# AlgoLab/rs-vgaligner

Measured on AMD Instinct MI355X. Metric: aligned reads/sec (10 kbp ONT vs HLA graph), higher is better.
Workload: dtype int32+f64

## Files before the change

rs-vgaligner_amd/csrc/vga_common.hpp:

```cpp
#pragma once

#include <hip/hip_runtime.h>
#include <sys/mman.h>

#include <chrono>
#include <cstdarg>
#include <cstdint>
#include <cstdio>
#include <cstdlib>
#include <cstring>
#include <atomic>
#include <memory>
#include <mutex>
#include <new>
#include <string>
#include <thread>
#include <vector>

#include "../../include/vga_hip.h"
#include "vga_probe_hash.hpp"

#define VGA_ABI_VERSION 6

template <typename T>
// ... 5 lines not shown
}

struct cov_state;
struct ps_state;
struct pu_state;
struct poa_ws;

struct vga_dev_index {
    uint32_t k = 0;
    uint64_t seq_length = 0;
    uint64_t n_nodes = 0, n_edges = 0;
    uint32_t *d_table = nullptr;
    uint64_t table_entries = 0;
    uint2 *d_pos = nullptr;
    uint64_t n_pos_words = 0;
    uint32_t *d_table_all = nullptr;
    uint2 *d_pos_all = nullptr;
    vga_hash_slot *d_hash = nullptr;
    uint32_t hash_mask = 0;
    bool all_view = false;
    uint64_t probe_table_bytes = 0, probe_pos_bytes = 0;
    char *d_seq_fwd = nullptr;
    uint32_t *d_node_start = nullptr, *d_edge_idx = nullptr, *d_edges_to = nullptr, *d_edges = nullptr;
    std::vector<char> seq_fwd;
    std::vector<uint32_t> node_start;
    std::vector<uint32_t> edge_idx;
    std::vector<uint32_t> edges_to;
    std::vector<uint32_t> edges;
    bool loaded = false;
    vga_owned<cov_state> cov{nullptr, nullptr};
    vga_owned<ps_state> ps{nullptr, nullptr};
    vga_owned<pu_state> pu{nullptr, nullptr};
};

struct vga_timer_entry {
    const char *name;
    hipEvent_t e0, e1;
    uint64_t bytes;
    hipStream_t stream;
};

struct vga_deferred { void *dev, *pinned, *reg; size_t reg_bytes; };

struct vga_ctx {
    int device = 0;
    hipStream_t stream = nullptr;
// ... 207 lines not shown
```

rs-vgaligner_amd/csrc/vga_ctx.hip:

```cpp
#include "vga_common.hpp"

#include <mutex>

#include <algorithm>

#include <malloc.h>

int vga_set_error(vga_ctx *ctx, int code, const char *fmt, ...)
{
    char buf[1024];
    va_list ap;
    va_start(ap, fmt);
    vsnprintf(buf, sizeof buf, fmt, ap);
    va_end(ap);
    if (ctx) { std::lock_guard<std::mutex> lk(ctx->err_mu); ctx->err = buf; }
    return code;
}

unsigned vga_host_threads(uint64_t n)
{
    unsigned nt = std::thread::hardware_concurrency();
    if (nt == 0) nt = 4;
    if (nt > 32) nt = 32;
    const char *e = getenv("VGA_HOST_THREADS");
// ... 93 lines not shown
    }
    vga_ctx *ctx = new vga_ctx();
    ctx->device = device;
    if (hipSetDevice(device) != hipSuccess) { delete ctx; return VGA_ERR_NO_DEVICE; }
    if (hipStreamCreateWithFlags(&ctx->stream, hipStreamNonBlocking) != hipSuccess) { delete ctx; return VGA_ERR_HIP; }
    hipDeviceProp_t prop;
    if (hipGetDeviceProperties(&prop, device) == hipSuccess) ctx->n_cu = prop.multiProcessorCount;
    *out = ctx;
    return VGA_OK;
}

void vga_index_release(vga_dev_index &ix)
{
    if (ix.d_table) (void)hipFree(ix.d_table);
    if (ix.d_pos) (void)hipFree(ix.d_pos);
    if (ix.d_table_all) (void)hipFree(ix.d_table_all);
    if (ix.d_pos_all) (void)hipFree(ix.d_pos_all);
    if (ix.d_hash) (void)hipFree(ix.d_hash);
    if (ix.d_seq_fwd) (void)hipFree(ix.d_seq_fwd);
    if (ix.d_node_start) (void)hipFree(ix.d_node_start);
    if (ix.d_edge_idx) (void)hipFree(ix.d_edge_idx);
    if (ix.d_edges_to) (void)hipFree(ix.d_edges_to);
    if (ix.d_edges) (void)hipFree(ix.d_edges);
    ix.cov.reset();
    ix.ps.reset();
    ix.pu.reset();
    ix = vga_dev_index();
}

extern "C" void vga_ctx_destroy(vga_ctx *ctx)
{
    if (!ctx) return;
    (void)hipSetDevice(ctx->device);
    vga_ctx_scope scope(ctx);
    if (ctx->stream) (void)hipStreamSynchronize(ctx->stream);
    for (vga_batch *b : ctx->batches) {
        if (b->d_reads) (void)hipFree(b->d_reads);
        if (b->d_read_off) (void)hipFree(b->d_read_off);
        if (b->d_read_off2) (void)hipFree(b->d_read_off2);
        b->d_reads = nullptr;
        b->d_read_off = nullptr;
        b->d_read_off2 = nullptr;
        b->ctx = nullptr;
    }
    ctx->map_ws.reset();
    ctx->poa_ws.reset();
// ... 129 lines not shown
    ix.seq_fwd.assign(d->seq_fwd, d->seq_fwd + d->seq_length);
    ix.node_start.resize(d->n_nodes + 1);
    ix.edge_idx.resize(d->n_nodes + 1);
    ix.edges_to.resize(d->n_nodes + 1);
    for (uint64_t i = 0; i <= d->n_nodes; i++) {
        ix.node_start[i] = (uint32_t)d->node_seq_idx[i];
        ix.edge_idx[i] = (uint32_t)d->node_edge_idx[i];
        ix.edges_to[i] = (uint32_t)d->node_edges_to[i];
    }
    ix.edges.resize(d->n_edges);
    for (uint64_t i = 0; i < d->n_edges; i++) ix.edges[i] = (uint32_t)d->edges[i];
    const size_t nn1 = (size_t)d->n_nodes + 1;
    VGA_HIP_CHECK(ctx, hipMalloc((void **)&ix.d_seq_fwd, d->seq_length + 16));
    VGA_HIP_CHECK(ctx, hipMalloc((void **)&ix.d_node_start, nn1 * sizeof(uint32_t)));
    VGA_HIP_CHECK(ctx, hipMalloc((void **)&ix.d_edge_idx, nn1 * sizeof(uint32_t)));
    VGA_HIP_CHECK(ctx, hipMalloc((void **)&ix.d_edges_to, nn1 * sizeof(uint32_t)));
    VGA_HIP_CHECK(ctx, hipMalloc((void **)&ix.d_edges, (d->n_edges + 1) * sizeof(uint32_t)));
    VGA_HIP_CHECK(ctx, hipMemcpyAsync(ix.d_seq_fwd, ix.seq_fwd.data(), d->seq_length, hipMemcpyHostToDevice, ctx->stream));
    VGA_HIP_CHECK(ctx, hipMemcpyAsync(ix.d_node_start, ix.node_start.data(), nn1 * sizeof(uint32_t), hipMemcpyHostToDevice, ctx->stream));
    VGA_HIP_CHECK(ctx, hipMemcpyAsync(ix.d_edge_idx, ix.edge_idx.data(), nn1 * sizeof(uint32_t), hipMemcpyHostToDevice, ctx->stream));
    VGA_HIP_CHECK(ctx, hipMemcpyAsync(ix.d_edges_to, ix.edges_to.data(), nn1 * sizeof(uint32_t), hipMemcpyHostToDevice, ctx->stream));
    if (d->n_edges)
        VGA_HIP_CHECK(ctx, hipMemcpyAsync(ix.d_edges, ix.edges.data(), d->n_edges * sizeof(uint32_t), hipMemcpyHostToDevice, ctx->stream));
    VGA_HIP_CHECK(ctx, hipStreamSynchronize(ctx->stream));
    return VGA_OK;
}

__global__ __launch_bounds__(256) void k_probe_hash_insert(const uint64_t *__restrict__ keys, const uint32_t *__restrict__ hdr_all,
                                                           const uint32_t *__restrict__ hdr_ff, uint64_t n, vga_hash_slot *slots,
                                                           uint32_t mask, uint32_t *n_failed)
{
    const uint64_t g = (uint64_t)blockIdx.x * blockDim.x + threadIdx.x;
    if (g >= n) return;
    const uint64_t key = keys[g];
    const uint32_t ha = hdr_all[g];
    uint32_t s = vga_hash_first_slot(key, mask);
    for (uint64_t tries = 0; tries <= mask; tries++, s = vga_hash_next_slot(s, mask)) {
        if (atomicCAS(&slots[s].hdr_all, VGA_HASH_EMPTY, ha) != VGA_HASH_EMPTY) continue;
        slots[s].key = key;
        slots[s].hdr_ff = hdr_ff[g];
        return;
    }
    atomicAdd(n_failed, 1u);
}

static int vga_index_upload_impl(vga_ctx *ctx, const vga_index_desc *d)
// ... 271 lines not shown
```

rs-vgaligner_amd/csrc/vga_subgraph.hip:

```cpp
#include "vga_subgraph.hpp"

#include <algorithm>
#include <string>
#include <vector>

namespace {

#define SG_RING_SPAN 32u

struct sg_index {
    const uint32_t *node_start, *edge_idx, *edges_to, *edges;
    const char *seq;
    uint32_t n_nodes;
};

__device__ __forceinline__ uint32_t sg_ld(const uint32_t *p) { return __hip_atomic_load(p, __ATOMIC_RELAXED, __HIP_MEMORY_SCOPE_AGENT); }

__device__ inline uint32_t sg_rank(const sg_index &ix, uint32_t pos)
{
    uint32_t lo = 0, hi = ix.n_nodes + 1;
    while (lo < hi) {
        const uint32_t mid = (lo + hi) >> 1;
        if (ix.node_start[mid] <= pos) lo = mid + 1; else hi = mid;
    }
    return lo;
}
__device__ inline uint32_t sg_select(const sg_index &ix, uint32_t element_no)
{
    if (element_no == 0 || element_no > ix.n_nodes + 1) return 0;
    return ix.node_start[element_no - 1];
}
__device__ inline uint32_t sg_len(const sg_index &ix, uint32_t h)
{
    const uint32_t id = h >> 1;
    return ix.node_start[id] - ix.node_start[id - 1];
}
template <typename F>
__device__ inline void sg_for_nb(const sg_index &ix, uint32_t h, bool incoming, F f)
{
    const uint32_t pos = (h >> 1) - 1;
    const bool inc = (h & 1u) ? !incoming : incoming;
    const uint32_t s0 = ix.edge_idx[pos], nin = ix.edges_to[pos];
    const uint32_t s = inc ? s0 : s0 + nin, e = inc ? s0 + nin : ix.edge_idx[pos + 1];
    const uint32_t fl = h & 1u;
    for (uint32_t i = s; i < e; i++) f(ix.edges[i] ^ fl);
}

__device__ inline bool sg_member(const uint32_t *bm, uint32_t nh, uint32_t x) { return x < nh && ((sg_ld(bm + (x >> 5)) >> (x & 31u)) & 1u); }

__device__ inline uint32_t wave_sum(uint32_t v)
{
#pragma unroll
    for (int o = 32; o > 0; o >>= 1) v += (uint32_t)__shfl_xor((int)v, o);
    return v;
}
__device__ inline uint32_t wave_max(uint32_t v)
{
#pragma unroll
    for (int o = 32; o > 0; o >>= 1) { const uint32_t t = (uint32_t)__shfl_xor((int)v, o); v = t > v ? t : v; }
    return v;
}
__device__ inline uint32_t wave_min(uint32_t v)
{
#pragma unroll
    for (int o = 32; o > 0; o >>= 1) { const uint32_t t = (uint32_t)__shfl_xor((int)v, o); v = t < v ? t : v; }
    return v;
}
__device__ inline unsigned long long wave_sum64(unsigned long long v)
{
#pragma unroll
    for (int o = 32; o > 0; o >>= 1)
        v += ((unsigned long long)(uint32_t)__shfl_xor((int)(v >> 32), o) << 32) | (uint32_t)__shfl_xor((int)(uint32_t)v, o);
    return v;
}
__device__ inline uint32_t wave_excl(uint32_t v, int lane, uint32_t *total)
{
    uint32_t s = v;
#pragma unroll
    for (int o = 1; o < 64; o <<= 1) {
        const uint32_t t = (uint32_t)__shfl_up((int)s, o);
        if (lane >= o) s += t;
    }
    *total = (uint32_t)__shfl((int)s, 63);
    return s - v;
}

struct sg_node_counts {
    uint32_t len, deg;
    bool has_out;
};
__device__ inline sg_node_counts sg_count_node(const sg_index &ix, const uint32_t *bm, uint32_t nh, uint32_t h)
{
    sg_node_counts c;
    c.len = sg_len(ix, h);
    c.deg = 0;
    c.has_out = false;
    sg_for_nb(ix, h, true, [&](uint32_t x) { if (x < h && sg_member(bm, nh, x)) c.deg++; });
    sg_for_nb(ix, h, false, [&](uint32_t y) { if (y > h && sg_member(bm, nh, y)) c.has_out = true; });
    return c;
}

__device__ void sg_extend(const sg_index &ix, uint32_t from, uint32_t diff, bool incoming, uint32_t *best, uint32_t *stamp,
                          uint32_t *q0, uint32_t *q1, uint32_t *touched, uint32_t &level, uint32_t *s_cnt, uint32_t *s_touched, int lane)
{
    auto relax = [&](uint32_t x, uint32_t rem, uint32_t lvl, uint32_t *q, uint32_t *qn) {
        const uint32_t old = atomicMax(best + x, rem);
        if (old < rem) {
            if (old == 0) touched[atomicAdd(s_touched, 1u)] = x;
            if (atomicExch(stamp + x, lvl) != lvl) q[atomicAdd(qn, 1u)] = x;
        }
    };
    if (lane == 0) { s_cnt[0] = 0; s_cnt[1] = 0; }
    __syncthreads();
    level++;
    if (lane == 0) sg_for_nb(ix, from, incoming, [&](uint32_t x) { relax(x, diff, level, q0, s_cnt); });
    int cq = 0;
    for (;;) {
        __syncthreads();
        const uint32_t cnt = s_cnt[cq];
        if (cnt == 0) break;
        __syncthreads();
        if (lane == 0) s_cnt[cq ^ 1] = 0;
        __syncthreads();
        level++;
        uint32_t *q = cq ? q1 : q0, *qo = cq ? q0 : q1;
        for (uint32_t i = (uint32_t)lane; i < cnt; i += 64) {
            const uint32_t h = sg_ld(q + i);
            const uint32_t left = sg_ld(best + h);
            const uint32_t len = sg_len(ix, h);
            if (len < left) {
                const uint32_t rem = left - len;
                sg_for_nb(ix, h, incoming, [&](uint32_t x) { relax(x, rem, level, qo, s_cnt + (cq ^ 1)); });
            }
        }
        cq ^= 1;
    }
}

__global__ __launch_bounds__(64) void k_sg_mark(const sg_desc *__restrict__ descs, uint32_t n, sg_index ix, uint32_t k, uint32_t words,
                                                uint32_t nh, uint32_t *bitmaps, uint32_t *scratch, sg_sum *sums)
{
    __shared__ uint32_t s_cnt[2], s_touched;
    const int lane = threadIdx.x;
    uint32_t *best = scratch + (uint64_t)blockIdx.x * 5ull * nh, *stamp = best + nh, *q0 = stamp + nh, *q1 = q0 + nh, *touched = q1 + nh;
    for (uint32_t i = (uint32_t)lane; i < nh; i += 64) { best[i] = 0; stamp[i] = 0; }
    uint32_t level = 0;
    __syncthreads();
    for (uint32_t p = blockIdx.x; p < n; p += gridDim.x) {
        const sg_desc d = descs[p];
        uint32_t *bm = bitmaps + (uint64_t)p * words;
        const uint32_t min_id = sg_rank(ix, d.pmin), max_id = sg_rank(ix, d.pmax);
        const uint32_t first_handle = min_id * 2, last_handle = max_id * 2;
        for (uint32_t w = (uint32_t)lane; w < words; w += 64) {
            const uint32_t lo = w * 32u, hi = lo + 31u;
            uint32_t m = 0;
            if (hi >= first_handle && lo <= last_handle) {
                m = 0x55555555u;
                if (first_handle > lo) m &= ~0u << (first_handle - lo);
                if (last_handle < hi) m &= ~0u >> (hi - last_handle);
            }
            bm[w] = m;
        }
        if (lane == 0) s_touched = 0;
        __syncthreads();
        uint32_t prefix_diff = d.q_first;
// ... 8 lines not shown
                atomicOr(bm + (h >> 5), 1u << (h & 31u));
                best[h] = 0;
                wlo = min(wlo, h >> 5);
                whi = max(whi, h >> 5);
            }
            __syncthreads();
            if (lane == 0) s_touched = 0;
            __syncthreads();
        };
        if (prefix_diff > 0) {
            sg_extend(ix, first_handle, prefix_diff, true, best, stamp, q0, q1, touched, level, s_cnt, &s_touched, lane);
            harvest();
        }
        uint32_t suffix_diff = d.qlen - (d.q_last + k);
        const uint32_t end_suffix_on_node = sg_select(ix, (last_handle >> 1) + 1) - 1 - (d.te_last - 1);
        if (end_suffix_on_node > suffix_diff) suffix_diff = 0; else suffix_diff -= end_suffix_on_node;
        if (suffix_diff > 0) {
            sg_extend(ix, last_handle, suffix_diff, false, best, stamp, q0, q1, touched, level, s_cnt, &s_touched, lane);
            harvest();
        }
        wlo = wave_min(wlo);
        whi = wave_max(whi);
        __syncthreads();
        uint32_t c_nodes = 0, c_preds = 0, c_sinks = 0, bad = 0;
        unsigned long long c_rows = 0;
        for (uint32_t w = wlo + (uint32_t)lane; w <= whi; w += 64) {
            uint32_t bits = sg_ld(bm + w);
            while (bits) {
                const uint32_t h = w * 32u + (uint32_t)__builtin_ctz(bits);
                bits &= bits - 1;
                const sg_node_counts c = sg_count_node(ix, bm, nh, h);
                c_nodes++;
                c_rows += c.len;
                c_preds += c.deg ? c.deg : 1u;
                c_sinks += c.has_out ? 0u : 1u;
                if (c.deg > 255 || c.len == 0 || c.len >= (1u << 24)) bad = 1;
            }
        }
        c_nodes = wave_sum(c_nodes);
        c_preds = wave_sum(c_preds);
        c_sinks = wave_sum(c_sinks);
        bad = wave_max(bad);
        const unsigned long long rows = wave_sum64(c_rows);
        if (rows >= (1ull << 31)) bad = 1;
        if (lane == 0) {
            sg_sum s = {};
            s.n_nodes = c_nodes; s.N = (uint32_t)rows; s.n_preds = c_preds; s.n_sinks = c_sinks; s.wlo = wlo; s.whi = whi; s.flags = bad;
            sums[p] = s;
        }
        __syncthreads();
    }
}

__device__ inline char sg_complement(char c)
{
    switch (c) {
    case 'a': return 't'; case 'c': return 'g'; case 't': return 'a'; case 'g': return 'c'; case 'u': return 'a';
    case 'A': return 'T'; case 'C': return 'G'; case 'T': return 'A'; case 'G': return 'C'; case 'U': return 'A';
    default: return 'N';
    }
}

__global__ __launch_bounds__(64) void k_sg_emit(uint32_t n, sg_index ix, uint32_t words, uint32_t nh, const uint32_t *bitmaps, uint32_t *scratch,
                                                sg_sum *sums, const sg_off *__restrict__ offs, uint32_t *handles, uint32_t *first_row, uint4 *ntab,
                                                uint32_t *preds, uint32_t *sinks, char *seq, int first_edge)
{
    const int lane = threadIdx.x;
    uint32_t *wb_rank = scratch + (uint64_t)blockIdx.x * 5ull * nh, *wb_row = wb_rank + words, *wb_pred = wb_row + words, *wb_sink = wb_pred + words;
    uint32_t *rf = scratch + (uint64_t)blockIdx.x * 5ull * nh + nh;
    for (uint32_t p = blockIdx.x; p < n; p += gridDim.x) {
        const sg_sum sm = sums[p];
        if (sm.flags & 1u) continue;
        const sg_off of = offs[p];
        const uint32_t *bm = bitmaps + (uint64_t)p * words;
        const uint32_t wlo = sm.wlo, whi = sm.whi, n_sub = sm.n_nodes;
        uint32_t *hd = handles + of.node0, *fr = first_row + of.node0, *pl = preds + of.pred0, *sl = sinks + of.sink0;
        uint4 *nt = ntab + of.node0 + p;
        char *sq = seq + of.seq0;
        {
            uint32_t run_rank = 0, run_row = 0, run_pred = 0, run_sink = 0;
            for (uint32_t w0 = wlo; w0 <= whi; w0 += 64) {
                const uint32_t w = w0 + (uint32_t)lane;
                uint32_t bits = w <= whi ? bm[w] : 0u;
                uint32_t cn = 0, cr = 0, cp = 0, cs = 0;
                while (bits) {
                    const uint32_t h = w * 32u + (uint32_t)__builtin_ctz(bits);
                    bits &= bits - 1;
                    const sg_node_counts c = sg_count_node(ix, bm, nh, h);
                    cn++; cr += c.len; cp += c.deg ? c.deg : 1u; cs += c.has_out ? 0u : 1u;
                }
                uint32_t tn, tr, tp, ts;
                const uint32_t en = wave_excl(cn, lane, &tn), er = wave_excl(cr, lane, &tr), ep = wave_excl(cp, lane, &tp), es = wave_excl(cs, lane, &ts);
                if (w <= whi) {
                    wb_rank[w - wlo] = run_rank + en; wb_row[w - wlo] = run_row + er; wb_pred[w - wlo] = run_pred + ep; wb_sink[w - wlo] = run_sink + es;
                }
                run_rank += tn; run_row += tr; run_pred += tp; run_sink += ts;
            }
        }
        __syncthreads();
        auto rank_of = [&](uint32_t x) -> uint32_t {
            const uint32_t w = x >> 5;
            return sg_ld(wb_rank + (w - wlo)) + (uint32_t)__builtin_popcount(bm[w] & ((1u << (x & 31u)) - 1u));
        };
        for (uint32_t w = wlo + (uint32_t)lane; w <= whi; w += 64) {
            uint32_t bits = bm[w];
            uint32_t i = sg_ld(wb_rank + (w - wlo)), row = sg_ld(wb_row + (w - wlo));
            while (bits) {
                const uint32_t h = w * 32u + (uint32_t)__builtin_ctz(bits);
                bits &= bits - 1;
                const uint32_t id = h >> 1, s = ix.node_start[id - 1], e = ix.node_start[id];
                hd[i] = h;
                fr[i] = row + 1;
                if (!(h & 1u)) for (uint32_t t = s; t < e; t++) sq[row + (t - s)] = ix.seq[t];
                else for (uint32_t t = e; t-- > s;) sq[row + (e - 1 - t)] = sg_complement(ix.seq[t]);
                row += e - s;
                i++;
            }
        }
        __syncthreads();
        uint32_t life = 1;
        for (uint32_t w = wlo + (uint32_t)lane; w <= whi; w += 64) {
            uint32_t bits = bm[w];
            uint32_t i = sg_ld(wb_rank + (w - wlo)), pcur = sg_ld(wb_pred + (w - wlo)), scur = sg_ld(wb_sink + (w - wlo));
            while (bits) {
                const uint32_t h = w * 32u + (uint32_t)__builtin_ctz(bits);
                bits &= bits - 1;
                const uint32_t len = sg_len(ix, h), frow = sg_ld(fr + i);
                uint32_t deg = 0, last_v = 0, last_k = 0, first_pred = 0;
                bool have_last = false;
                for (;;) {
                    uint32_t best_v = 0xFFFFFFFFu, best_k = 0xFFFFFFFFu, kk = 0;
                    sg_for_nb(ix, h, true, [&](uint32_t x) {
                        const uint32_t kx = kk++;
                        if (!(x < h && sg_member(bm, nh, x))) return;
                        if (have_last && (x < last_v || (x == last_v && kx <= last_k))) return;
                        if (x < best_v || (x == best_v && kx < best_k)) { best_v = x; best_k = kx; }
                    });
                    if (best_k == 0xFFFFFFFFu) break;
                    const uint32_t r = rank_of(best_v);
                    const uint32_t lrow = sg_ld(fr + r) + sg_len(ix, best_v) - 1;
                    pl[pcur + deg] = lrow;
                    if (deg == 0) first_pred = lrow;
                    deg++;
                    last_v = best_v; last_k = best_k; have_last = true;
                }
                if (deg == 0) pl[pcur] = 0;
                uint32_t reach = 0;
                bool has_out = false;
                sg_for_nb(ix, h, false, [&](uint32_t y) {
                    if (y > h && sg_member(bm, nh, y)) { has_out = true; const uint32_t sp = rank_of(y) - i; reach = sp > reach ? sp : reach; }
                });
                if (!has_out) sl[scur++] = frow + len - 1;
                if (reach <= SG_RING_SPAN) life = reach > life ? reach : life;
                nt[1 + i] = make_uint4(frow, len | ((deg ? deg : 1u) << 24), (has_out ? 0u : 0x80000000u) | (reach > SG_RING_SPAN ? 0x40000000u : 0u),
                                       deg <= 1 ? first_pred : pcur);
                pcur += deg ? deg : 1u;
                i++;
            }
        }
        life = wave_max(life);
        __syncthreads();
        uint32_t longest = 0, first_src = 0xFFFFFFFFu;
        for (uint32_t g0 = 0; g0 < n_sub; g0 += 64) {
            const uint32_t top = n_sub - 1 - g0;
            const bool valid = (uint32_t)lane <= top;
            const uint32_t i = valid ? top - (uint32_t)lane : 0u;
            uint32_t val = 0, len = 1;
            unsigned long long mask = 0;
            if (valid) {
                const uint32_t h = sg_ld(hd + i);
                len = sg_len(ix, h);
                bool taken = false;
                sg_for_nb(ix, h, false, [&](uint32_t y) {
                    if (!(y > h && sg_member(bm, nh, y))) return;
                    if (first_edge && taken) return;
                    taken = true;
                    const uint32_t j = rank_of(y);
                    if (j > top) { const uint32_t c = 1u + sg_ld(rf + j); val = c > val ? c : val; }
                    else mask |= 1ull << (top - j);
                });
            }
            for (int s = 0; s < 64; s++) {
                const uint32_t rfs = (uint32_t)__shfl((int)(val + len - 1), s);
                if ((mask >> s) & 1ull) { const uint32_t c = 1u + rfs; val = c > val ? c : val; }
            }
            if (valid) {
                rf[i] = val + len - 1;
                uint32_t *z = (uint32_t *)(nt + 1 + i);
                const uint32_t y = sg_ld(z + 1), wv = sg_ld(z + 3), zf = sg_ld(z + 2);
                z[2] = zf | val;
                if ((y >> 24) == 1u && wv == 0u) {
                    const uint32_t c = 1u + val + len - 1;
                    if (first_edge) { if (i < first_src) { first_src = i; longest = c; } }
                    else longest = c > longest ? c : longest;
                }
            }
            __syncthreads();
        }
        if (first_edge) {
            const uint32_t fs = wave_min(first_src);
            longest = wave_max(first_src == fs && fs != 0xFFFFFFFFu ? longest : 0u);
        } else
            longest = wave_max(longest);
        if (lane == 0) {
            nt[0] = make_uint4(0u, 1u, longest, 0u);
            sums[p].longest = longest;
            sums[p].life = life;
            if (longest >= (1u << 30)) sums[p].flags = 1u;
        }
        __syncthreads();
    }
}

struct sg_part_bufs {
    vga_dbuf<uint32_t> d_handles, d_first_row, d_preds, d_sinks;
    vga_dbuf<uint4> d_ntab;
    vga_dbuf<char> d_seq;
    vga_hbuf<uint32_t> h_handles, h_first_row;
};
struct sg_ws {
    vga_dbuf<sg_desc> d_desc;
    vga_dbuf<sg_sum> d_sum;
    vga_dbuf<sg_off> d_off;
    vga_dbuf<uint32_t> d_bitmaps, d_scratch;
    vga_hbuf<sg_desc> h_desc;
    vga_hbuf<sg_sum> h_sum;
    vga_hbuf<sg_off> h_off;
    sg_part_bufs part[2];
    std::vector<uint64_t> q_src;
    std::string dump;
    std::vector<uint64_t> read_no;
    hipStream_t side = nullptr;
    uint64_t waves = 0;
    uint32_t nh = 0, words = 0;
    ~sg_ws()
    {
        if (side) (void)hipStreamDestroy(side);
    }
};

int sg_dump_part(vga_ctx *ctx, sg_ws &W, const sg_part_bufs &B, uint64_t p0, uint64_t p1, uint64_t tn, uint64_t tp, uint64_t ts, uint64_t tq, hipStream_t st)
{
    const uint64_t n = p1 - p0;
    std::vector<uint4> ntab(tn + n);
    std::vector<uint32_t> preds(tp + 1), sinks(ts + 1);
    std::vector<char> seq(tq + 4);
    VGA_HIP_CHECK_OOM(ctx, hipMemcpyAsync(ntab.data(), B.d_ntab.p, (tn + n) * sizeof(uint4), hipMemcpyDeviceToHost, st));
    if (tp) VGA_HIP_CHECK_OOM(ctx, hipMemcpyAsync(preds.data(), B.d_preds.p, tp * sizeof(uint32_t), hipMemcpyDeviceToHost, st));
    if (ts) VGA_HIP_CHECK_OOM(ctx, hipMemcpyAsync(sinks.data(), B.d_sinks.p, ts * sizeof(uint32_t), hipMemcpyDeviceToHost, st));
    if (tq) VGA_HIP_CHECK_OOM(ctx, hipMemcpyAsync(seq.data(), B.d_seq.p, tq, hipMemcpyDeviceToHost, st));
    VGA_HIP_CHECK_OOM(ctx, hipStreamSynchronize(st));
    FILE *f = fopen(W.dump.c_str(), "a");
    if (!f) return vga_set_error(ctx, VGA_ERR_ARG, "VGA_SG_DUMP: cannot append to %s", W.dump.c_str());
    auto list = [&](const char *tag, const uint32_t *v, uint64_t cnt) {
        fputs(tag, f);
        for (uint64_t i = 0; i < cnt; i++) fprintf(f, " %u", v[i]);
        fputc('\n', f);
// ... 8 lines not shown
        if (s.flags & 1u) continue;
        const uint4 *nt = ntab.data() + o.node0 + (p - p0);
        for (uint32_t i = 0; i <= s.n_nodes; i++)
            fprintf(f, "T %u %u %u %u %u %u %u %u\n", i, nt[i].x, nt[i].y & 0xFFFFFFu, nt[i].y >> 24, nt[i].z >> 31, (nt[i].z >> 30) & 1u, nt[i].z & 0x3FFFFFFFu, nt[i].w);
        list("H", B.h_handles.p + o.node0, s.n_nodes);
        list("F", B.h_first_row.p + o.node0, s.n_nodes);
        list("L", preds.data() + o.pred0, s.n_preds);
        list("K", sinks.data() + o.sink0, s.n_sinks);
        fputs("Q ", f);
        for (uint32_t i = 0; i < s.N; i++) fprintf(f, "%02x", (unsigned)(unsigned char)seq[o.seq0 + i]);
        fputs("\nE\n", f);
    }
    fclose(f);
    return VGA_OK;
}

int sg_run_part(vga_ctx *ctx, sg_ws &W, sg_store &store, int k, uint64_t p0, uint64_t p1, hipStream_t st)
{
    sg_part &P = store.part[k];
    P.p0 = p0; P.p1 = p1;
    if (p1 <= p0) { P.ready = true; return VGA_OK; }
    const uint64_t n = p1 - p0;
    const vga_dev_index &dix = ctx->index;
    sg_index ix = {dix.d_node_start, dix.d_edge_idx, dix.d_edges_to, dix.d_edges, dix.d_seq_fwd, (uint32_t)dix.n_nodes};
    const uint32_t nh = W.nh, words = W.words;
    uint32_t waves = (uint32_t)std::min<uint64_t>(W.waves, n);
    if (k == 1) {
        uint32_t side_waves = 2u * (uint32_t)ctx->n_cu;
        if (const char *e = getenv("VGA_SG_SIDE_WAVES")) side_waves = (uint32_t)std::max(1, atoi(e));
        waves = std::min(waves, side_waves);
    }
    sg_part_bufs &B = W.part[k];
    int t_mark = vga_timer_begin(ctx, "subgraph_mark", 0, st);
    hipLaunchKernelGGL(k_sg_mark, dim3(waves), dim3(64), 0, st, W.d_desc.p + p0, (uint32_t)n, ix, dix.k, words, nh, W.d_bitmaps.p + p0 * words,
                       W.d_scratch.p, W.d_sum.p + p0);
    vga_timer_end(ctx, t_mark);
    VGA_HIP_CHECK_OOM(ctx, hipGetLastError());
    VGA_HIP_CHECK_OOM(ctx, hipMemcpyAsync(W.h_sum.p + p0, W.d_sum.p + p0, n * sizeof(sg_sum), hipMemcpyDeviceToHost, st));
    VGA_HIP_CHECK_OOM(ctx, hipStreamSynchronize(st));
    uint64_t tn = 0, tp = 0, ts = 0, tq = 0;
    for (uint64_t p = p0; p < p1; p++) {
        const sg_sum &s = W.h_sum.p[p];
        sg_off &o = W.h_off.p[p];
        o.node0 = tn; o.pred0 = tp; o.sink0 = ts; o.seq0 = tq; o.q_src = W.q_src[p];
        if (s.flags & 1u) continue;
        tn += s.n_nodes; tp += s.n_preds; ts += s.n_sinks; tq += ((uint64_t)s.N + 3) & ~3ull;
    }
    VGA_HIP_CHECK_OOM(ctx, B.d_handles.reserve(tn + 1)); VGA_HIP_CHECK_OOM(ctx, B.d_first_row.reserve(tn + 1)); VGA_HIP_CHECK_OOM(ctx, B.d_ntab.reserve(tn + n));
    VGA_HIP_CHECK_OOM(ctx, B.d_preds.reserve(tp + 1)); VGA_HIP_CHECK_OOM(ctx, B.d_sinks.reserve(ts + 1)); VGA_HIP_CHECK_OOM(ctx, B.d_seq.reserve(tq + 4));
    VGA_HIP_CHECK_OOM(ctx, B.h_handles.reserve(tn + 1)); VGA_HIP_CHECK_OOM(ctx, B.h_first_row.reserve(tn + 1));
    VGA_HIP_CHECK_OOM(ctx, hipMemcpyAsync(W.d_off.p + p0, W.h_off.p + p0, n * sizeof(sg_off), hipMemcpyHostToDevice, st));
    int t_emit = vga_timer_begin(ctx, "subgraph_emit", 0, st);
    hipLaunchKernelGGL(k_sg_emit, dim3(waves), dim3(64), 0, st, (uint32_t)n, ix, words, nh, W.d_bitmaps.p + p0 * words, W.d_scratch.p, W.d_sum.p + p0,
                       W.d_off.p + p0, B.d_handles.p, B.d_first_row.p, B.d_ntab.p, B.d_preds.p, B.d_sinks.p, B.d_seq.p,
                       store.remain_rule == VGA_REMAIN_FIRST_OUT_EDGE ? 1 : 0);
    vga_timer_end(ctx, t_emit);
    VGA_HIP_CHECK_OOM(ctx, hipGetLastError());
    VGA_HIP_CHECK_OOM(ctx, hipMemcpyAsync(W.h_sum.p + p0, W.d_sum.p + p0, n * sizeof(sg_sum), hipMemcpyDeviceToHost, st));
    if (tn) {
        VGA_HIP_CHECK_OOM(ctx, hipMemcpyAsync(B.h_handles.p, B.d_handles.p, tn * sizeof(uint32_t), hipMemcpyDeviceToHost, st));
        VGA_HIP_CHECK_OOM(ctx, hipMemcpyAsync(B.h_first_row.p, B.d_first_row.p, tn * sizeof(uint32_t), hipMemcpyDeviceToHost, st));
    }
    VGA_HIP_CHECK_OOM(ctx, hipStreamSynchronize(st));
    if (!W.dump.empty()) {
        const int rc = sg_dump_part(ctx, W, B, p0, p1, tn, tp, ts, tq, st);
        if (rc != VGA_OK) return rc;
    }
    P.d_ntab = B.d_ntab.p; P.d_preds = B.d_preds.p; P.d_sinks = B.d_sinks.p; P.d_seq = B.d_seq.p;
    P.d_handles = B.d_handles.p;
    P.h_handles = B.h_handles.p; P.h_first_row = B.h_first_row.p;
    P.ready = true;
    return VGA_OK;
}

}

int sg_prepare(vga_ctx *ctx, const sg_desc *descs, const uint64_t *q_src, const uint64_t *read_no, uint64_t n, uint64_t split, const char *d_reads,
               int remain_rule, sg_store &store)
// ... 3 lines not shown
    if (n == 0) return VGA_OK;
    if (n >= (1ull << 31)) return vga_set_error(ctx, VGA_ERR_UNSUPPORTED, "too many chains in one call");
    (void)hipSetDevice(ctx->device);
    hipStream_t st = ctx->stream;
    if (!ctx->sg_ws && !(ctx->sg_ws = vga_make_owned<void, sg_ws>())) throw std::bad_alloc();
    sg_ws &W = *(sg_ws *)ctx->sg_ws.get();
    if (!W.side) {
        int lo = 0, hi = 0;
        (void)hipDeviceGetStreamPriorityRange(&lo, &hi);
        (void)hi;
        VGA_HIP_CHECK_OOM(ctx, hipStreamCreateWithPriority(&W.side, hipStreamNonBlocking, lo));
    }
    const vga_dev_index &dix = ctx->index;
    W.nh = 2u * ((uint32_t)dix.n_nodes + 2u);
    W.words = (W.nh + 31u) / 32u;
    uint64_t waves = std::min<uint64_t>(n, 16ull * (uint64_t)ctx->n_cu);
    const uint64_t slab = 5ull * W.nh * sizeof(uint32_t);
    W.waves = std::max<uint64_t>(1, std::min<uint64_t>(waves, (4ull << 30) / slab));
    if (split > n) split = n;
    VGA_HIP_CHECK_OOM(ctx, W.d_desc.reserve(n)); VGA_HIP_CHECK_OOM(ctx, W.d_sum.reserve(n)); VGA_HIP_CHECK_OOM(ctx, W.d_off.reserve(n));
    VGA_HIP_CHECK_OOM(ctx, W.h_desc.reserve(n)); VGA_HIP_CHECK_OOM(ctx, W.h_sum.reserve(n)); VGA_HIP_CHECK_OOM(ctx, W.h_off.reserve(n));
    VGA_HIP_CHECK_OOM(ctx, W.d_bitmaps.reserve(n * W.words));
    VGA_HIP_CHECK_OOM(ctx, W.d_scratch.reserve(W.waves * 5ull * W.nh));
    memcpy(W.h_desc.p, descs, n * sizeof(sg_desc));
    W.q_src.assign(q_src, q_src + n);
    const char *dump = getenv("VGA_SG_DUMP");
    W.dump = dump ? dump : "";
    if (!W.dump.empty()) {
        W.read_no.assign(read_no, read_no + n);
        FILE *f = fopen(W.dump.c_str(), "w");
        if (!f) return vga_set_error(ctx, VGA_ERR_ARG, "VGA_SG_DUMP: cannot write %s", W.dump.c_str());
        fclose(f);
    }
    VGA_HIP_CHECK_OOM(ctx, hipMemcpyAsync(W.d_desc.p, W.h_desc.p, n * sizeof(sg_desc), hipMemcpyHostToDevice, st));
    store.n = n;
    store.split = split;
    store.sum = W.h_sum.p; store.off = W.h_off.p; store.d_off = W.d_off.p;
    store.d_reads = d_reads;
    store.part[1].p0 = split; store.part[1].p1 = n;
    return sg_run_part(ctx, W, store, 0, 0, split, st);
}

int sg_prepare_rest(vga_ctx *ctx, sg_store &store)
{
    if (store.part[1].ready) return VGA_OK;
    (void)hipSetDevice(ctx->device);
// ... 4 lines not shown
```

Measured before the change: 10610.

## Pack per-node records, cache bitmap window in LDS, reuse mark prefix sums in emit

Builds a packed 16-byte per-node record (length and edge ranges) and a presorted incoming-edge list at index load, so each node's data comes from one vector load and predecessor emission can scan sorted edges instead of repeatedly searching for the minimum. The mark kernel stages the subgraph bitmap window in shared memory and writes per-word prefix counts to a side buffer, which the emit kernel reuses rather than recounting. Emit also splits sequence copying into a separate coalesced word-wise pass and caches single-successor ranks for the reach pass. The cost is extra device memory for the side buffer and tables, plus a fallback path for windows that exceed the shared-memory size.

Result: no change. 10620 (median of 2 runs) (+0.1%).

```diff
diff --git a/rs-vgaligner_amd/csrc/vga_common.hpp b/rs-vgaligner_amd/csrc/vga_common.hpp
--- a/rs-vgaligner_amd/csrc/vga_common.hpp
+++ b/rs-vgaligner_amd/csrc/vga_common.hpp
@@ -51,6 +51,8 @@
     uint64_t probe_table_bytes = 0, probe_pos_bytes = 0;
     char *d_seq_fwd = nullptr;
     uint32_t *d_node_start = nullptr, *d_edge_idx = nullptr, *d_edges_to = nullptr, *d_edges = nullptr;
+    uint4 *d_sg_rec = nullptr;
+    uint32_t *d_edges_in_sorted = nullptr;
     std::vector<char> seq_fwd;
     std::vector<uint32_t> node_start;
     std::vector<uint32_t> edge_idx;
diff --git a/rs-vgaligner_amd/csrc/vga_ctx.hip b/rs-vgaligner_amd/csrc/vga_ctx.hip
--- a/rs-vgaligner_amd/csrc/vga_ctx.hip
+++ b/rs-vgaligner_amd/csrc/vga_ctx.hip
@@ -1,4 +1,5 @@
 #include "vga_common.hpp"
+#include "vga_sg_tables.hpp"
 
 #include <mutex>
 
@@ -139,6 +140,8 @@
     if (ix.d_edge_idx) (void)hipFree(ix.d_edge_idx);
     if (ix.d_edges_to) (void)hipFree(ix.d_edges_to);
     if (ix.d_edges) (void)hipFree(ix.d_edges);
+    if (ix.d_sg_rec) (void)hipFree(ix.d_sg_rec);
+    if (ix.d_edges_in_sorted) (void)hipFree(ix.d_edges_in_sorted);
     ix.cov.reset();
     ix.ps.reset();
     ix.pu.reset();
@@ -314,6 +317,15 @@
     VGA_HIP_CHECK(ctx, hipMemcpyAsync(ix.d_edges_to, ix.edges_to.data(), nn1 * sizeof(uint32_t), hipMemcpyHostToDevice, ctx->stream));
     if (d->n_edges)
         VGA_HIP_CHECK(ctx, hipMemcpyAsync(ix.d_edges, ix.edges.data(), d->n_edges * sizeof(uint32_t), hipMemcpyHostToDevice, ctx->stream));
+    if (ix.edge_idx[d->n_nodes] > d->n_edges) return vga_set_error(ctx, VGA_ERR_ARG, "node_edge_idx runs past the %llu edges", (unsigned long long)d->n_edges);
+    std::vector<sg_node_rec> rec(d->n_nodes + 1);
+    std::vector<uint32_t> in_sorted(d->n_edges + 1);
+    sg_build_tables(ix.node_start.data(), ix.edge_idx.data(), ix.edges_to.data(), ix.edges.data(), d->n_nodes, rec.data(), in_sorted.data());
+    static_assert(sizeof(sg_node_rec) == sizeof(uint4), "one 16-byte load per node");
+    VGA_HIP_CHECK(ctx, hipMalloc((void **)&ix.d_sg_rec, (d->n_nodes + 1) * sizeof(uint4)));
+    VGA_HIP_CHECK(ctx, hipMalloc((void **)&ix.d_edges_in_sorted, (d->n_edges + 1) * sizeof(uint32_t)));
+    VGA_HIP_CHECK(ctx, hipMemcpyAsync(ix.d_sg_rec, rec.data(), (d->n_nodes + 1) * sizeof(uint4), hipMemcpyHostToDevice, ctx->stream));
+    VGA_HIP_CHECK(ctx, hipMemcpyAsync(ix.d_edges_in_sorted, in_sorted.data(), (d->n_edges + 1) * sizeof(uint32_t), hipMemcpyHostToDevice, ctx->stream));
     VGA_HIP_CHECK(ctx, hipStreamSynchronize(ctx->stream));
     return VGA_OK;
 }
diff --git a/rs-vgaligner_amd/csrc/vga_sg_tables.hpp b/rs-vgaligner_amd/csrc/vga_sg_tables.hpp
--- /dev/null
+++ b/rs-vgaligner_amd/csrc/vga_sg_tables.hpp
@@ -0,0 +1,19 @@
+#pragma once
+
+#include <algorithm>
+#include <cstdint>
+
+struct sg_node_rec {
+    uint32_t len, e_in, e_out, e_end;
+};
+
+inline void sg_build_tables(const uint32_t *node_start, const uint32_t *edge_idx, const uint32_t *edges_to, const uint32_t *edges, uint64_t n_nodes,
+                            sg_node_rec *rec, uint32_t *in_sorted)
+{
+    for (uint64_t i = 0; i < n_nodes; i++) {
+        const uint32_t s0 = edge_idx[i], end = edge_idx[i + 1], mid = std::min(s0 + edges_to[i], end);
+        rec[i] = sg_node_rec{node_start[i + 1] - node_start[i], s0, mid, end};
+        std::copy(edges + s0, edges + end, in_sorted + s0);
+        std::sort(in_sorted + s0, in_sorted + mid);
+    }
+}
diff --git a/rs-vgaligner_amd/csrc/vga_subgraph.hip b/rs-vgaligner_amd/csrc/vga_subgraph.hip
--- a/rs-vgaligner_amd/csrc/vga_subgraph.hip
+++ b/rs-vgaligner_amd/csrc/vga_subgraph.hip
@@ -8,8 +8,14 @@
 
 #define SG_RING_SPAN 32u
 
+#define SG_WINDOW 1024u
+#define SG_SIDE_BYTES (128ull << 20)
+#define SG_NONE 0xFFFFFFFFu
+#define SG_MULTI 0x80000000u
+
 struct sg_index {
-    const uint32_t *node_start, *edge_idx, *edges_to, *edges;
+    const uint32_t *node_start, *edges, *edges_in_sorted;
+    const uint4 *rec;
     const char *seq;
     uint32_t n_nodes;
 };
@@ -30,23 +36,26 @@
     if (element_no == 0 || element_no > ix.n_nodes + 1) return 0;
     return ix.node_start[element_no - 1];
 }
-__device__ inline uint32_t sg_len(const sg_index &ix, uint32_t h)
-{
-    const uint32_t id = h >> 1;
-    return ix.node_start[id] - ix.node_start[id - 1];
-}
+__device__ inline uint4 sg_rec(const sg_index &ix, uint32_t h) { return ix.rec[(h >> 1) - 1]; }
 template <typename F>
-__device__ inline void sg_for_nb(const sg_index &ix, uint32_t h, bool incoming, F f)
-{
-    const uint32_t pos = (h >> 1) - 1;
+__device__ inline void sg_for_nb(const sg_index &ix, const uint4 &r, uint32_t h, bool incoming, F f)
+{
     const bool inc = (h & 1u) ? !incoming : incoming;
-    const uint32_t s0 = ix.edge_idx[pos], nin = ix.edges_to[pos];
-    const uint32_t s = inc ? s0 : s0 + nin, e = inc ? s0 + nin : ix.edge_idx[pos + 1];
+    const uint32_t s = inc ? r.y : r.z, e = inc ? r.z : r.w;
     const uint32_t fl = h & 1u;
     for (uint32_t i = s; i < e; i++) f(ix.edges[i] ^ fl);
 }
 
-__device__ inline bool sg_member(const uint32_t *bm, uint32_t nh, uint32_t x) { return x < nh && ((sg_ld(bm + (x >> 5)) >> (x & 31u)) & 1u); }
+struct sg_set {
+    const uint32_t *bm, *win;
+    uint32_t wlo, whi, nh;
+    __device__ inline uint32_t word(uint32_t w) const { return win ? win[w - wlo] : sg_ld(bm + w); }
+    __device__ inline bool has(uint32_t x) const
+    {
+        const uint32_t w = x >> 5;
+        return x < nh && w >= wlo && w <= whi && ((word(w) >> (x & 31u)) & 1u);
+    }
+};
 
 __device__ inline uint32_t wave_sum(uint32_t v)
 {
@@ -89,14 +98,34 @@
     uint32_t len, deg;
     bool has_out;
 };
-__device__ inline sg_node_counts sg_count_node(const sg_index &ix, const uint32_t *bm, uint32_t nh, uint32_t h)
-{
+__device__ inline sg_node_counts sg_count_node(const sg_index &ix, const sg_set &set, uint32_t h)
+{
+    const uint4 r = sg_rec(ix, h);
     sg_node_counts c;
-    c.len = sg_len(ix, h);
+    c.len = r.x;
     c.deg = 0;
     c.has_out = false;
-    sg_for_nb(ix, h, true, [&](uint32_t x) { if (x < h && sg_member(bm, nh, x)) c.deg++; });
-    sg_for_nb(ix, h, false, [&](uint32_t y) { if (y > h && sg_member(bm, nh, y)) c.has_out = true; });
+    sg_for_nb(ix, r, h, true, [&](uint32_t x) { if (x < h && set.has(x)) c.deg++; });
+    sg_for_nb(ix, r, h, false, [&](uint32_t y) { if (y > h && set.has(y)) c.has_out = true; });
+    return c;
+}
+struct sg_word_counts {
+    uint32_t n, rows, preds, sinks, bad;
+};
+__device__ inline sg_word_counts sg_count_word(const sg_index &ix, const sg_set &set, uint32_t w)
+{
+    sg_word_counts c = {0, 0, 0, 0, 0};
+    uint32_t bits = w <= set.whi ? set.word(w) : 0u;
+    while (bits) {
+        const uint32_t h = w * 32u + (uint32_t)__builtin_ctz(bits);
+        bits &= bits - 1;
+        const sg_node_counts k = sg_count_node(ix, set, h);
+        c.n++;
+        c.rows += k.len;
+        c.preds += k.deg ? k.deg : 1u;
+        c.sinks += k.has_out ? 0u : 1u;
+        if (k.deg > 255 || k.len == 0 || k.len >= (1u << 24)) c.bad = 1;
+    }
     return c;
 }
 
@@ -113,7 +142,7 @@
     if (lane == 0) { s_cnt[0] = 0; s_cnt[1] = 0; }
     __syncthreads();
     level++;
-    if (lane == 0) sg_for_nb(ix, from, incoming, [&](uint32_t x) { relax(x, diff, level, q0, s_cnt); });
+    if (lane == 0) sg_for_nb(ix, sg_rec(ix, from), from, incoming, [&](uint32_t x) { relax(x, diff, level, q0, s_cnt); });
     int cq = 0;
     for (;;) {
         __syncthreads();
@@ -127,10 +156,11 @@
         for (uint32_t i = (uint32_t)lane; i < cnt; i += 64) {
             const uint32_t h = sg_ld(q + i);
             const uint32_t left = sg_ld(best + h);
-            const uint32_t len = sg_len(ix, h);
+            const uint4 r = sg_rec(ix, h);
+            const uint32_t len = r.x;
             if (len < left) {
                 const uint32_t rem = left - len;
-                sg_for_nb(ix, h, incoming, [&](uint32_t x) { relax(x, rem, level, qo, s_cnt + (cq ^ 1)); });
+                sg_for_nb(ix, r, h, incoming, [&](uint32_t x) { relax(x, rem, level, qo, s_cnt + (cq ^ 1)); });
             }
         }
         cq ^= 1;
@@ -138,9 +168,10 @@
 }
 
 __global__ __launch_bounds__(64) void k_sg_mark(const sg_desc *__restrict__ descs, uint32_t n, sg_index ix, uint32_t k, uint32_t words,
-                                                uint32_t nh, uint32_t *bitmaps, uint32_t *scratch, sg_sum *sums)
+                                                uint32_t nh, uint32_t *bitmaps, uint32_t *scratch, sg_sum *sums, uint32_t win, uint4 *side)
 {
     __shared__ uint32_t s_cnt[2], s_touched;
+    __shared__ uint32_t s_bm[SG_WINDOW];
     const int lane = threadIdx.x;
     uint32_t *best = scratch + (uint64_t)blockIdx.x * 5ull * nh, *stamp = best + nh, *q0 = stamp + nh, *q1 = q0 + nh, *touched = q1 + nh;
     for (uint32_t i = (uint32_t)lane; i < nh; i += 64) { best[i] = 0; stamp[i] = 0; }
@@ -195,20 +226,27 @@
         wlo = wave_min(wlo);
         whi = wave_max(whi);
         __syncthreads();
+        const bool fits = whi - wlo < win;
+        if (fits) {
+            for (uint32_t w = wlo + (uint32_t)lane; w <= whi; w += 64) s_bm[w - wlo] = sg_ld(bm + w);
+            __syncthreads();
+        }
+        const sg_set set = {bm, fits ? s_bm : nullptr, wlo, whi, nh};
+        uint4 *wb = side + (uint64_t)p * win;
         uint32_t c_nodes = 0, c_preds = 0, c_sinks = 0, bad = 0;
         unsigned long long c_rows = 0;
-        for (uint32_t w = wlo + (uint32_t)lane; w <= whi; w += 64) {
-            uint32_t bits = sg_ld(bm + w);
-            while (bits) {
-                const uint32_t h = w * 32u + (uint32_t)__builtin_ctz(bits);
-                bits &= bits - 1;
-                const sg_node_counts c = sg_count_node(ix, bm, nh, h);
-                c_nodes++;
-                c_rows += c.len;
-                c_preds += c.deg ? c.deg : 1u;
-                c_sinks += c.has_out ? 0u : 1u;
-                if (c.deg > 255 || c.len == 0 || c.len >= (1u << 24)) bad = 1;
-            }
+        uint4 run = make_uint4(0u, 0u, 0u, 0u);
+        for (uint32_t w0 = wlo; w0 <= whi; w0 += 64) {
+            const uint32_t w = w0 + (uint32_t)lane;
+            const sg_word_counts c = sg_count_word(ix, set, w);
+            c_nodes += c.n; c_rows += c.rows; c_preds += c.preds; c_sinks += c.sinks; bad |= c.bad;
+            if (fits) {
+                uint32_t tn, tr, tp, ts;
+                const uint32_t en = wave_excl(c.n, lane, &tn), er = wave_excl(c.rows, lane, &tr), ep = wave_excl(c.preds, lane, &tp), es = wave_excl(c.sinks, lane, &ts);
+                if (w <= whi) wb[w - wlo] = make_uint4(run.x + en, run.y + er, run.z + ep, run.w + es);
+                run.x += tn; run.y += tr; run.z += tp; run.w += ts;
+            }
+            if (w0 + 64 < w0) break;
         }
         c_nodes = wave_sum(c_nodes);
         c_preds = wave_sum(c_preds);
@@ -234,13 +272,33 @@
     }
 }
 
+__device__ inline void sg_copy_run(const char *src, char *dst, uint32_t len, int lane)
+{
+    uint32_t head = (4u - (uint32_t)((uintptr_t)dst & 3u)) & 3u;
+    if (head > len) head = len;
+    if ((uint32_t)lane < head) dst[lane] = src[lane];
+    src += head; dst += head; len -= head;
+    const uint32_t nd = len >> 2, sa = (uint32_t)((uintptr_t)src & 3u);
+    const uint32_t *s32 = (const uint32_t *)(src - sa);
+    uint32_t *d32 = (uint32_t *)dst;
+    for (uint32_t k = (uint32_t)lane; k < nd; k += 64) {
+        const uint32_t lo = s32[k], hi = sa ? s32[k + 1] : 0u;
+        d32[k] = (uint32_t)((((unsigned long long)hi << 32) | lo) >> (8u * sa));
+    }
+    const uint32_t tail = len & 3u;
+    if ((uint32_t)lane < tail) dst[4u * nd + (uint32_t)lane] = src[4u * nd + (uint32_t)lane];
+}
+
 __global__ __launch_bounds__(64) void k_sg_emit(uint32_t n, sg_index ix, uint32_t words, uint32_t nh, const uint32_t *bitmaps, uint32_t *scratch,
                                                 sg_sum *sums, const sg_off *__restrict__ offs, uint32_t *handles, uint32_t *first_row, uint4 *ntab,
-                                                uint32_t *preds, uint32_t *sinks, char *seq, int first_edge)
-{
+                                                uint32_t *preds, uint32_t *sinks, char *seq, int first_edge, uint32_t win, const uint4 *side)
+{
+    __shared__ uint32_t s_bm[SG_WINDOW], s_rank[SG_WINDOW];
     const int lane = threadIdx.x;
-    uint32_t *wb_rank = scratch + (uint64_t)blockIdx.x * 5ull * nh, *wb_row = wb_rank + words, *wb_pred = wb_row + words, *wb_sink = wb_pred + words;
-    uint32_t *rf = scratch + (uint64_t)blockIdx.x * 5ull * nh + nh;
+    uint32_t *slab = scratch + (uint64_t)blockIdx.x * 5ull * nh;
+    uint32_t *wb_own = slab;
+    uint32_t *rf = slab + nh;
+    uint32_t *sx = slab + 2ull * nh;
     for (uint32_t p = blockIdx.x; p < n; p += gridDim.x) {
         const sg_sum sm = sums[p];
         if (sm.flags & 1u) continue;
@@ -250,79 +308,123 @@
         uint32_t *hd = handles + of.node0, *fr = first_row + of.node0, *pl = preds + of.pred0, *sl = sinks + of.sink0;
         uint4 *nt = ntab + of.node0 + p;
         char *sq = seq + of.seq0;
-        {
-            uint32_t run_rank = 0, run_row = 0, run_pred = 0, run_sink = 0;
+        const bool fits = whi - wlo < win;
+        const sg_set set = {bm, fits ? s_bm : nullptr, wlo, whi, nh};
+        const uint32_t *wb = fits ? (const uint32_t *)(side + (uint64_t)p * win) : wb_own;
+        if (fits) {
+            for (uint32_t w = wlo + (uint32_t)lane; w <= whi; w += 64) { s_bm[w - wlo] = bm[w]; s_rank[w - wlo] = wb[4u * (w - wlo)]; }
+        } else {
+            uint4 run = make_uint4(0u, 0u, 0u, 0u);
             for (uint32_t w0 = wlo; w0 <= whi; w0 += 64) {
                 const uint32_t w = w0 + (uint32_t)lane;
-                uint32_t bits = w <= whi ? bm[w] : 0u;
-                uint32_t cn = 0, cr = 0, cp = 0, cs = 0;
-                while (bits) {
-                    const uint32_t h = w * 32u + (uint32_t)__builtin_ctz(bits);
-                    bits &= bits - 1;
-                    const sg_node_counts c = sg_count_node(ix, bm, nh, h);
-                    cn++; cr += c.len; cp += c.deg ? c.deg : 1u; cs += c.has_out ? 0u : 1u;
+                const sg_word_counts c = sg_count_word(ix, set, w);
+                uint32_t tn, tr, tp, ts;
+                const uint32_t en = wave_excl(c.n, lane, &tn), er = wave_excl(c.rows, lane, &tr), ep = wave_excl(c.preds, lane, &tp), es = wave_excl(c.sinks, lane, &ts);
+                if (w <= whi) {
+                    uint32_t *o = wb_own + 4u * (w - wlo);
+                    o[0] = run.x + en; o[1] = run.y + er; o[2] = run.z + ep; o[3] = run.w + es;
                 }
-                uint32_t tn, tr, tp, ts;
-                const uint32_t en = wave_excl(cn, lane, &tn), er = wave_excl(cr, lane, &tr), ep = wave_excl(cp, lane, &tp), es = wave_excl(cs, lane, &ts);
-                if (w <= whi) {
-                    wb_rank[w - wlo] = run_rank + en; wb_row[w - wlo] = run_row + er; wb_pred[w - wlo] = run_pred + ep; wb_sink[w - wlo] = run_sink + es;
-                }
-                run_rank += tn; run_row += tr; run_pred += tp; run_sink += ts;
-            }
-        }
-        __syncthreads();
+                run.x += tn; run.y += tr; run.z += tp; run.w += ts;
+                if (w0 + 64 < w0) break;
+            }
+        }
+        __syncthreads();
+        auto wb_at = [&](uint32_t w, int c) -> uint32_t { return sg_ld(wb + 4u * (w - wlo) + c); };
         auto rank_of = [&](uint32_t x) -> uint32_t {
             const uint32_t w = x >> 5;
-            return sg_ld(wb_rank + (w - wlo)) + (uint32_t)__builtin_popcount(bm[w] & ((1u << (x & 31u)) - 1u));
+            return (fits ? s_rank[w - wlo] : wb_at(w, 0)) + (uint32_t)__builtin_popcount(set.word(w) & ((1u << (x & 31u)) - 1u));
         };
         for (uint32_t w = wlo + (uint32_t)lane; w <= whi; w += 64) {
-            uint32_t bits = bm[w];
-            uint32_t i = sg_ld(wb_rank + (w - wlo)), row = sg_ld(wb_row + (w - wlo));
+            uint32_t bits = set.word(w);
+            uint32_t i = wb_at(w, 0), row = wb_at(w, 1);
             while (bits) {
                 const uint32_t h = w * 32u + (uint32_t)__builtin_ctz(bits);
                 bits &= bits - 1;
-                const uint32_t id = h >> 1, s = ix.node_start[id - 1], e = ix.node_start[id];
                 hd[i] = h;
                 fr[i] = row + 1;
-                if (!(h & 1u)) for (uint32_t t = s; t < e; t++) sq[row + (t - s)] = ix.seq[t];
-                else for (uint32_t t = e; t-- > s;) sq[row + (e - 1 - t)] = sg_complement(ix.seq[t]);
-                row += e - s;
+                row += sg_rec(ix, h).x;
                 i++;
             }
         }
         __syncthreads();
+        for (uint32_t g0 = 0; g0 < n_sub; g0 += 64) {
+            const uint32_t i = g0 + (uint32_t)lane;
+            const bool valid = i < n_sub;
+            uint32_t h = 0, row = 0, len = 0, start = 0;
+            if (valid) {
+                h = sg_ld(hd + i);
+                row = sg_ld(fr + i) - 1u;
+                len = (i + 1 < n_sub ? sg_ld(fr + i + 1) - 1u : sm.N) - row;
+                start = ix.node_start[(h >> 1) - 1];
+            }
+            const uint32_t hprev = (uint32_t)__shfl_up((int)h, 1);
+            const bool fwd = valid && !(h & 1u);
+            const bool cont = fwd && lane > 0 && hprev + 2u == h;
+            const unsigned long long m_cont = __ballot(cont), m_valid = __ballot(valid);
+            unsigned long long heads = __ballot(fwd && !cont);
+            const int nv = __popcll(m_valid);
+            while (heads) {
+                const int s = __builtin_ctzll(heads);
+                heads &= heads - 1;
+                const unsigned long long stop = s == 63 ? 0ull : (~m_cont) >> (s + 1);
+                const int e = stop ? s + 1 + __builtin_ctzll(stop) : 64;
+                const uint32_t r0 = (uint32_t)__shfl((int)row, s), src0 = (uint32_t)__shfl((int)start, s);
+                const uint32_t r_next = (uint32_t)__shfl((int)row, e < nv ? e : 0), r_last = (uint32_t)__shfl((int)(row + len), nv - 1);
+                sg_copy_run(ix.seq + src0, sq + r0, (e < nv ? r_next : r_last) - r0, lane);
+            }
+            if (valid && (h & 1u)) {
+                const uint32_t e = start + len;
+                for (uint32_t t = e; t-- > start;) sq[row + (e - 1 - t)] = sg_complement(ix.seq[t]);
+            }
+        }
         uint32_t life = 1;
         for (uint32_t w = wlo + (uint32_t)lane; w <= whi; w += 64) {
-            uint32_t bits = bm[w];
-            uint32_t i = sg_ld(wb_rank + (w - wlo)), pcur = sg_ld(wb_pred + (w - wlo)), scur = sg_ld(wb_sink + (w - wlo));
+            uint32_t bits = set.word(w);
+            uint32_t i = wb_at(w, 0), pcur = wb_at(w, 2), scur = wb_at(w, 3);
             while (bits) {
                 const uint32_t h = w * 32u + (uint32_t)__builtin_ctz(bits);
                 bits &= bits - 1;
-                const uint32_t len = sg_len(ix, h), frow = sg_ld(fr + i);
-                uint32_t deg = 0, last_v = 0, last_k = 0, first_pred = 0;
-                bool have_last = false;
-                for (;;) {
-                    uint32_t best_v = 0xFFFFFFFFu, best_k = 0xFFFFFFFFu, kk = 0;
-                    sg_for_nb(ix, h, true, [&](uint32_t x) {
-                        const uint32_t kx = kk++;
-                        if (!(x < h && sg_member(bm, nh, x))) return;
-                        if (have_last && (x < last_v || (x == last_v && kx <= last_k))) return;
-                        if (x < best_v || (x == best_v && kx < best_k)) { best_v = x; best_k = kx; }
-                    });
-                    if (best_k == 0xFFFFFFFFu) break;
-                    const uint32_t r = rank_of(best_v);
-                    const uint32_t lrow = sg_ld(fr + r) + sg_len(ix, best_v) - 1;
+                const uint4 r = sg_rec(ix, h);
+                const uint32_t len = r.x, frow = sg_ld(fr + i);
+                uint32_t deg = 0, first_pred = 0;
+                auto put = [&](uint32_t x) {
+                    const uint32_t lrow = sg_ld(fr + rank_of(x) + 1) - 1u;
                     pl[pcur + deg] = lrow;
                     if (deg == 0) first_pred = lrow;
                     deg++;
-                    last_v = best_v; last_k = best_k; have_last = true;
+                };
+                if (!(h & 1u)) {
+                    for (uint32_t t = r.y; t < r.z; t++) {
+                        const uint32_t x = ix.edges_in_sorted[t];
+                        if (x >= h) break;
+                        if (set.has(x)) put(x);
+                    }
+                } else {
+                    uint32_t last_v = 0, last_k = 0;
+                    bool have_last = false;
+                    for (;;) {
+                        uint32_t best_v = 0xFFFFFFFFu, best_k = 0xFFFFFFFFu, kk = 0;
+                        sg_for_nb(ix, r, h, true, [&](uint32_t x) {
+                            const uint32_t kx = kk++;
+                            if (!(x < h && set.has(x))) return;
+                            if (have_last && (x < last_v || (x == last_v && kx <= last_k))) return;
+                            if (x < best_v || (x == best_v && kx < best_k)) { best_v = x; best_k = kx; }
+                        });
+                        if (best_k == 0xFFFFFFFFu) break;
+                        put(best_v);
+                        last_v = best_v; last_k = best_k; have_last = true;
+                    }
                 }
                 if (deg == 0) pl[pcur] = 0;
-                uint32_t reach = 0;
-                bool has_out = false;
-                sg_for_nb(ix, h, false, [&](uint32_t y) {
-                    if (y > h && sg_member(bm, nh, y)) { has_out = true; const uint32_t sp = rank_of(y) - i; reach = sp > reach ? sp : reach; }
+                uint32_t reach = 0, succ = SG_NONE;
+                sg_for_nb(ix, r, h, false, [&](uint32_t y) {
+                    if (!(y > h && set.has(y))) return;
+                    const uint32_t j = rank_of(y), sp = j - i;
+                    reach = sp > reach ? sp : reach;
+                    succ = succ == SG_NONE ? j : succ | SG_MULTI;
                 });
+                const bool has_out = succ != SG_NONE;
+                sx[i] = succ;
                 if (!has_out) sl[scur++] = frow + len - 1;
                 if (reach <= SG_RING_SPAN) life = reach > life ? reach : life;
                 nt[1 + i] = make_uint4(frow, len | ((deg ? deg : 1u) << 24), (has_out ? 0u : 0x80000000u) | (reach > SG_RING_SPAN ? 0x40000000u : 0u),
@@ -340,18 +442,20 @@
             const uint32_t i = valid ? top - (uint32_t)lane : 0u;
             uint32_t val = 0, len = 1;
             unsigned long long mask = 0;
+            uint32_t *z = (uint32_t *)(nt + 1 + i);
             if (valid) {
-                const uint32_t h = sg_ld(hd + i);
-                len = sg_len(ix, h);
-                bool taken = false;
-                sg_for_nb(ix, h, false, [&](uint32_t y) {
-                    if (!(y > h && sg_member(bm, nh, y))) return;
-                    if (first_edge && taken) return;
-                    taken = true;
-                    const uint32_t j = rank_of(y);
+                len = sg_ld(z + 1) & 0xFFFFFFu;
+                auto take = [&](uint32_t j) {
                     if (j > top) { const uint32_t c = 1u + sg_ld(rf + j); val = c > val ? c : val; }
                     else mask |= 1ull << (top - j);
-                });
+                };
+                const uint32_t succ = sg_ld(sx + i);
+                if (succ == SG_NONE) {
+                } else if (first_edge || !(succ & SG_MULTI)) take(succ & ~SG_MULTI);
+                else {
+                    const uint32_t h = sg_ld(hd + i);
+                    sg_for_nb(ix, sg_rec(ix, h), h, false, [&](uint32_t y) { if (y > h && set.has(y)) take(rank_of(y)); });
+                }
             }
             for (int s = 0; s < 64; s++) {
                 const uint32_t rfs = (uint32_t)__shfl((int)(val + len - 1), s);
@@ -359,7 +463,6 @@
             }
             if (valid) {
                 rf[i] = val + len - 1;
-                uint32_t *z = (uint32_t *)(nt + 1 + i);
                 const uint32_t y = sg_ld(z + 1), wv = sg_ld(z + 3), zf = sg_ld(z + 2);
                 z[2] = zf | val;
                 if ((y >> 24) == 1u && wv == 0u) {
@@ -396,6 +499,7 @@
     vga_dbuf<sg_sum> d_sum;
     vga_dbuf<sg_off> d_off;
     vga_dbuf<uint32_t> d_bitmaps, d_scratch;
+    vga_dbuf<uint4> d_side;
     vga_hbuf<sg_desc> h_desc;
     vga_hbuf<sg_sum> h_sum;
     vga_hbuf<sg_off> h_off;
@@ -405,7 +509,7 @@
     std::vector<uint64_t> read_no;
     hipStream_t side = nullptr;
     uint64_t waves = 0;
-    uint32_t nh = 0, words = 0;
+    uint32_t nh = 0, words = 0, win = 0;
     ~sg_ws()
     {
         if (side) (void)hipStreamDestroy(side);
@@ -460,7 +564,7 @@
     if (p1 <= p0) { P.ready = true; return VGA_OK; }
     const uint64_t n = p1 - p0;
     const vga_dev_index &dix = ctx->index;
-    sg_index ix = {dix.d_node_start, dix.d_edge_idx, dix.d_edges_to, dix.d_edges, dix.d_seq_fwd, (uint32_t)dix.n_nodes};
+    sg_index ix = {dix.d_node_start, dix.d_edges, dix.d_edges_in_sorted, dix.d_sg_rec, dix.d_seq_fwd, (uint32_t)dix.n_nodes};
     const uint32_t nh = W.nh, words = W.words;
     uint32_t waves = (uint32_t)std::min<uint64_t>(W.waves, n);
     if (k == 1) {
@@ -471,7 +575,7 @@
     sg_part_bufs &B = W.part[k];
     int t_mark = vga_timer_begin(ctx, "subgraph_mark", 0, st);
     hipLaunchKernelGGL(k_sg_mark, dim3(waves), dim3(64), 0, st, W.d_desc.p + p0, (uint32_t)n, ix, dix.k, words, nh, W.d_bitmaps.p + p0 * words,
-                       W.d_scratch.p, W.d_sum.p + p0);
+                       W.d_scratch.p, W.d_sum.p + p0, W.win, W.d_side.p + p0 * W.win);
     vga_timer_end(ctx, t_mark);
     VGA_HIP_CHECK_OOM(ctx, hipGetLastError());
     VGA_HIP_CHECK_OOM(ctx, hipMemcpyAsync(W.h_sum.p + p0, W.d_sum.p + p0, n * sizeof(sg_sum), hipMemcpyDeviceToHost, st));
@@ -491,7 +595,7 @@
     int t_emit = vga_timer_begin(ctx, "subgraph_emit", 0, st);
     hipLaunchKernelGGL(k_sg_emit, dim3(waves), dim3(64), 0, st, (uint32_t)n, ix, words, nh, W.d_bitmaps.p + p0 * words, W.d_scratch.p, W.d_sum.p + p0,
                        W.d_off.p + p0, B.d_handles.p, B.d_first_row.p, B.d_ntab.p, B.d_preds.p, B.d_sinks.p, B.d_seq.p,
-                       store.remain_rule == VGA_REMAIN_FIRST_OUT_EDGE ? 1 : 0);
+                       store.remain_rule == VGA_REMAIN_FIRST_OUT_EDGE ? 1 : 0, W.win, W.d_side.p + p0 * W.win);
     vga_timer_end(ctx, t_emit);
     VGA_HIP_CHECK_OOM(ctx, hipGetLastError());
     VGA_HIP_CHECK_OOM(ctx, hipMemcpyAsync(W.h_sum.p + p0, W.d_sum.p + p0, n * sizeof(sg_sum), hipMemcpyDeviceToHost, st));
@@ -541,6 +645,9 @@
     VGA_HIP_CHECK_OOM(ctx, W.h_desc.reserve(n)); VGA_HIP_CHECK_OOM(ctx, W.h_sum.reserve(n)); VGA_HIP_CHECK_OOM(ctx, W.h_off.reserve(n));
     VGA_HIP_CHECK_OOM(ctx, W.d_bitmaps.reserve(n * W.words));
     VGA_HIP_CHECK_OOM(ctx, W.d_scratch.reserve(W.waves * 5ull * W.nh));
+    W.win = (uint32_t)std::min<uint64_t>(SG_WINDOW, SG_SIDE_BYTES / sizeof(uint4) / n);
+    if (const char *e = getenv("VGA_SG_WINDOW")) W.win = std::min(W.win, (uint32_t)std::max(0, atoi(e)));
+    VGA_HIP_CHECK_OOM(ctx, W.d_side.reserve(n * W.win + 1));
     memcpy(W.h_desc.p, descs, n * sizeof(sg_desc));
     W.q_src.assign(q_src, q_src + n);
     const char *dump = getenv("VGA_SG_DUMP");
```
